# flyakon/DeepPhysiNet

Hardware: AMD Instinct MI355X
Metric: collocation-points/sec (fwd+PDE-Jacobian+bwd) (higher is better)
Workload: dtype bf16x2 (hi+lo split bf16 MFMA operands), fp32 accumulate

## Files before the change

### deepphysinet_amd/csrc/dpn_layout.h

```cpp
#pragma once

#if defined(__HIPCC__)
#define DPN_HD __host__ __device__ constexpr
#else
#define DPN_HD constexpr
#endif

namespace dpn {

constexpr int kNets = 6;
constexpr int kHidden = 256;
constexpr int kPe = 192;
constexpr int kW1Stride = 193;
constexpr int kW2Stride = 257;

DPN_HD int drow32(int r, int h) { return (r & 3) + 8 * (r >> 2) + 4 * h; }
DPN_HD int chain_ch(int ks, int h, int e) { return 16 * ks + 8 * (e >> 2) + 4 * h + (e & 3); }

DPN_HD int pe3_angle(int ks, int h, int e) { return 8 * ks + 4 * h + (e >> 1); }
DPN_HD int pe3_ch(int ks, int h, int e) { return (pe3_angle(ks, h, e) & 31) * 6 + (e & 1) * 3 + (pe3_angle(ks, h, e) >> 5); }
DPN_HD int pe6_ch(int ks, int h, int e) { return (pe3_angle(ks, h, e) & 15) * 12 + (e & 1) * 6 + (pe3_angle(ks, h, e) >> 4); }

DPN_HD int gpe_row_to_pe3_ch(int rho) {
    const int T = rho >> 5, i = rho & 31;
    const int r = (i & 3) + 4 * (i >> 3), h = (i >> 2) & 1;
    return pe3_ch(2 * T + (r >> 3), h, r & 7);
}

constexpr int kS0 = 0;
constexpr int kS1 = kS0 + 8 * 12;
constexpr int kS2 = kS1 + 8 * 28;
constexpr int kS3 = kS2 + 8 * 16;
constexpr int kS4 = kS3 + 8 * 16;
constexpr int kS5 = kS4 + 8 * 16;
constexpr int kPackKB = kS5 + 6 * 16;
enum { kVecB1 = 0, kVecCvec, kVecBf1, kVecU, kVecWo, kVecB2BdE_unused, kNumVecs = 6 };
DPN_HD long pack_bytes_per_net(int ns) { return (long)kPackKB * 1024 * ns + kNumVecs * 1024 + 16; }

constexpr int kF0 = kS0, kFA = kS1, kFB = kS1 + 8 * 16, kFAT = kS2, kF5 = kS5;
static_assert(kFB + 8 * 12 == kS2 && kFAT + 8 * 16 == kS3, "fused form fits the block");
enum { kVecC2 = kVecCvec, kVecA2 = kVecBf1, kVecBv = kVecB2BdE_unused };

}
```

### deepphysinet_amd/csrc/dpn_wgrad.hip

```cpp
#include "dpn_point_common.h"

DEV u16 f2bf(float x) {
    unsigned u = __float_as_uint(x);
    u += 0x7FFFu + ((u >> 16) & 1u);
    return (u16)(u >> 16);
}
DEV float bf2f(u16 b) { return __uint_as_float(((unsigned)b) << 16); }

struct PackArgs {
    DpnNetPtrs net[kNets];
    char* packed;
    int ns;
    int form;
    int n_fields;
    long heads_stride, evec_stride, packed_stride;
};
DEV DpnNetPtrs pack_net(const PackArgs& a, const int net, const int field) {
    DpnNetPtrs P = a.net[net];
    P.w1b1 += field * a.heads_stride;
    P.w2b2 += field * a.heads_stride;
    P.evec += field * a.evec_stride;
    return P;
}

DEV float pack_src(const DpnNetPtrs& P, int kb, int lane, int e) {
    const int i = lane & 31, h = lane >> 5;
    if (kb < kS1) {
        const int T = kb / 12, ks = kb % 12;
        return P.w1b1[(32 * T + i) * P.ld_w1b1 + pe3_ch(ks, h, e)];
    } else if (kb >= kS5) {
        const int rel = kb - kS5, T = rel / 16, ks = rel % 16;
        return P.w1b1[chain_ch(ks, h, e) * P.ld_w1b1 + gpe_row_to_pe3_ch(32 * T + i)];
    }
    if (kb < kS2) {
        const int rel = kb - kS1;
        if (rel < 128) return P.w2b2[(32 * (rel / 16) + i) * P.ld_w2b2 + chain_ch(rel % 16, h, e)];
        const int r2 = rel - 128;
        return P.Wd[(32 * (r2 / 12) + i) * kPe + pe6_ch(r2 % 12, h, e)];
    } else if (kb < kS3) {
        const int rel = kb - kS2, T = rel / 16, ks = rel % 16;
        return P.W1[(32 * T + i) * kHidden + chain_ch(ks, h, e)];
    } else if (kb < kS4) {
        const int rel = kb - kS3, T = rel / 16, ks = rel % 16;
        return P.W1[chain_ch(ks, h, e) * kHidden + (32 * T + i)];
    } else {
        const int rel = kb - kS4, T = rel / 16, ks = rel % 16;
        return P.w2b2[chain_ch(ks, h, e) * P.ld_w2b2 + (32 * T + i)];
    }
}

constexpr int kVecParts = 8;
DEV void pack_vectors(const PackArgs& a, const DpnNetPtrs& P, char* packed_net, const int part) {
    float* vec = reinterpret_cast<float*>(packed_net + (long)kPackKB * 1024 * a.ns);
    const int tid = threadIdx.x, og = tid >> 5;
    const int idx = 32 * part + (tid & 31);
    const int h = idx >> 7, T = (idx >> 4) & 7, r = idx & 15;
    const int ch = 32 * T + drow32(r, h);
    const int c6 = idx < kPe ? pe6_ch(idx >> 4, (idx >> 3) & 1, idx & 7) : 0;
    __shared__ float red[3][8][32];
    float up = 0.f, a2 = 0.f, bv = 0.f;
    if (a.form == 1) {
#pragma unroll 8
        for (int o = 32 * og; o < 32 * og + 32; ++o) {
            const float w = P.wo[o];
            up = fmaf(w, P.W2[o * kHidden + ch], up);
            a2 = fmaf(w, P.w2b2[o * P.ld_w2b2 + ch], a2);
            bv = fmaf(w, P.Wd[o * kPe + c6], bv);
        }
    } else {
#pragma unroll 8
        for (int o = 32 * og; o < 32 * og + 32; ++o) up = fmaf(P.wo[o], P.W2[o * kHidden + ch], up);
    }
    red[0][og][tid & 31] = up; red[1][og][tid & 31] = a2; red[2][og][tid & 31] = bv;
    __syncthreads();
    if (og == 0) {
        const int c = tid;
        auto sum8 = [&](const int q) { return ((red[q][0][c] + red[q][1][c]) + (red[q][2][c] + red[q][3][c])) + ((red[q][4][c] + red[q][5][c]) + (red[q][6][c] + red[q][7][c])); };
        vec[kVecB1 * 256 + idx] = P.w1b1[ch * P.ld_w1b1 + kPe];
        vec[kVecU * 256 + idx] = sum8(0);
        vec[kVecWo * 256 + idx] = P.wo[ch];
        if (a.form == 1) {
            vec[kVecA2 * 256 + idx] = sum8(1);
            vec[kVecBv * 256 + idx] = idx < kPe ? sum8(2) : 0.f;
        } else {
            vec[kVecCvec * 256 + idx] = P.w2b2[ch * P.ld_w2b2 + kHidden] + P.bd[ch] + P.evec[ch];
            vec[kVecBf1 * 256 + idx] = P.bf1[ch];
            vec[kVecB2BdE_unused * 256 + idx] = 0.f;
        }
    }
    if (part != 0) return;
    __shared__ float red1[256];
    const float cv_nat = P.w2b2[tid * P.ld_w2b2 + kHidden] + P.bd[tid] + P.evec[tid];
    red1[tid] = P.wo[tid] * (P.bf2[tid] + (a.form == 1 ? 2.0f * cv_nat : 0.f));
    __syncthreads();
    for (int s = 128; s > 0; s >>= 1) {
        if (tid < s) red1[tid] += red1[tid + s];
        __syncthreads();
    }
    if (tid == 0) {
        vec[kNumVecs * 256 + 0] = red1[0] + P.bo[0];
        vec[kNumVecs * 256 + 1] = (float)a.form; vec[kNumVecs * 256 + 2] = 0.f; vec[kNumVecs * 256 + 3] = 0.f;
    }
}

__global__ __launch_bounds__(256) void dpn_pack_matrices_kernel(PackArgs a) {
    const int mcols = gridDim.x - kVecParts;
    const int field = blockIdx.y / kNets, net = blockIdx.y - field * kNets;
    const int ns = a.ns;
    const DpnNetPtrs P = pack_net(a, net, field);
    char* packed_net = a.packed + field * a.packed_stride + (long)net * pack_bytes_per_net(ns);
    if ((int)blockIdx.x >= mcols) { pack_vectors(a, P, packed_net, blockIdx.x - mcols); return; }
    uint4* dst = reinterpret_cast<uint4*>(packed_net);
    const int total = kPackKB * 64;
    for (int u = blockIdx.x * 256 + threadIdx.x; u < total; u += mcols * 256) {
        const int kb = u >> 6;
        const int lane = u & 63;
        u16 hi[8], lo[8];
#pragma unroll
        for (int e = 0; e < 8; ++e) {
            const float x = pack_src(P, kb, lane, e);
            hi[e] = f2bf(x);
            lo[e] = f2bf(x - bf2f(hi[e]));
        }
        uint4 w;
        w.x = hi[0] | (hi[1] << 16); w.y = hi[2] | (hi[3] << 16); w.z = hi[4] | (hi[5] << 16); w.w = hi[6] | (hi[7] << 16);
        dst[(kb * ns) * 64 + lane] = w;
        if (ns == 2) {
            w.x = lo[0] | (lo[1] << 16); w.y = lo[2] | (lo[3] << 16); w.z = lo[4] | (lo[5] << 16); w.w = lo[6] | (lo[7] << 16);
            dst[(kb * ns + 1) * 64 + lane] = w;
        }
    }
}

constexpr int kFusedBlocks = 64 + 48 + 8 + 12 + kVecParts;
DEV f32x16 pk_mfma_f32(float a, float b, f32x16 c) { return __builtin_amdgcn_mfma_f32_32x32x2f32(a, b, c, 0, 0, 0); }
__global__ __launch_bounds__(256) void dpn_pack_fused_kernel(PackArgs a) {
#ifdef PACK_NO_XCD_REMAP
    const int field = blockIdx.y / kNets, net = blockIdx.y - field * kNets, bx = blockIdx.x, ns = a.ns;
#else
    const int lin = blockIdx.x + kFusedBlocks * blockIdx.y, virt = (lin & 7) * (kFusedBlocks * kNets / 8 * a.n_fields) + (lin >> 3);
    static_assert(kFusedBlocks * kNets % 8 == 0, "remap");
    const int fnet = virt / kFusedBlocks, bx = virt - fnet * kFusedBlocks, ns = a.ns, field = fnet / kNets, net = fnet - field * kNets;
#endif
#ifdef PACK_ABL_MASK
    if (!((PACK_ABL_MASK >> (bx < 64 ? 0 : bx < 112 ? 1 : bx < 120 ? 2 : bx < 132 ? 3 : 4)) & 1)) return;
#endif
    const DpnNetPtrs P = pack_net(a, net, field);
    char* packed_net = a.packed + field * a.packed_stride + (long)net * pack_bytes_per_net(ns);
    if (bx >= 132) { pack_vectors(a, P, packed_net, bx - 132); return; }
    uint4* dst = reinterpret_cast<uint4*>(packed_net);
    auto put = [&](const int kb, const int lane, const float (&x)[8]) __attribute__((always_inline)) {
        u16 hi[8], lo[8];
#pragma unroll
        for (int e = 0; e < 8; ++e) { hi[e] = f2bf(x[e]); lo[e] = f2bf(x[e] - bf2f(hi[e])); }
        uint4 w;
        w.x = hi[0] | (hi[1] << 16); w.y = hi[2] | (hi[3] << 16); w.z = hi[4] | (hi[5] << 16); w.w = hi[6] | (hi[7] << 16);
        dst[(kb * ns) * 64 + lane] = w;
        if (ns == 2) {
            w.x = lo[0] | (lo[1] << 16); w.y = lo[2] | (lo[3] << 16); w.z = lo[4] | (lo[5] << 16); w.w = lo[6] | (lo[7] << 16);
            dst[(kb * ns + 1) * 64 + lane] = w;
        }
    };
    if (bx >= 120) {
        for (int u = (bx - 120) * 256 + threadIdx.x; u < 192 * 64; u += 12 * 256) {
            int kb = u >> 6;
            const int lane = u & 63;
            if (kb >= kS1) kb += kS5 - kS1;
            float x[8];
#pragma unroll
            for (int e = 0; e < 8; ++e) x[e] = pack_src(P, kb, lane, e);
            put(kb, lane, x);
        }
        return;
    }
    const int role = bx < 64 ? 0 : bx < 112 ? 1 : 2;
    const int rb = role == 0 ? bx : role == 1 ? bx - 64 : bx - 112;
    const int To = rb & 7, Tc = role == 2 ? 0 : rb >> 3;
    const int lane = threadIdx.x & 63, wv = threadIdx.x >> 6, col = lane & 31, kh = lane >> 5;
    __shared__ float red[4][16][64];
    __shared__ float tile[32][33];
    const float* W1r = P.W1 + (32 * To + col) * kHidden;
    int ccol = 0;
    if (role == 0) ccol = 32 * Tc + col;
    else if (role == 1) { const int sl = 32 * Tc + col; ccol = pe6_ch(sl >> 4, (sl >> 3) & 1, sl & 7); }
    f32x16 acc = (f32x16)0.f;
    float av[32], bv[32];
#pragma unroll
    for (int m = 0; m < 8; ++m) {
        const int k0 = 64 * wv + 8 * m + 4 * kh;
        const f32x4 q = *reinterpret_cast<const f32x4*>(W1r + k0);
#pragma unroll
        for (int e = 0; e < 4; ++e) {
            const int k = k0 + e;
            av[4 * m + e] = q[e];
            if (role == 0) bv[4 * m + e] = P.w2b2[(long)k * P.ld_w2b2 + ccol];
            else if (role == 1) bv[4 * m + e] = P.Wd[k * kPe + ccol];
            else bv[4 * m + e] = col == 0 ? (P.w2b2[(long)k * P.ld_w2b2 + kHidden] + P.bd[k] + P.evec[k]) : 0.f;
        }
    }
#pragma unroll
    for (int kk = 0; kk < 32; ++kk) acc = pk_mfma_f32(av[kk], bv[kk], acc);
#pragma unroll
    for (int r = 0; r < 16; ++r) red[wv][r][lane] = acc[r];
    __syncthreads();
#pragma unroll
    for (int q = 0; q < 4; ++q) {
        const int r = wv + 4 * q;
        tile[drow32(r, kh)][col] = (red[0][r][lane] + red[1][r][lane]) + (red[2][r][lane] + red[3][r][lane]);
    }
    __syncthreads();
    if (role == 2) {
        if (threadIdx.x < 32) {
            const int o = 32 * To + threadIdx.x, w_ = o & 31;
            float* vec = reinterpret_cast<float*>(packed_net + (long)kPackKB * 1024 * ns);
            vec[kVecC2 * 256 + ((w_ >> 2) & 1) * 128 + (o >> 5) * 16 + (w_ & 3) + 4 * (w_ >> 3)] = tile[threadIdx.x][0] + P.bf1[o];
        }
        return;
    }
    const int form = threadIdx.x >> 7, ksl = (threadIdx.x >> 6) & 1, i = lane & 31, h = lane >> 5;
    float x[8];
    if (role == 1) {
        if (form == 1) return;
#pragma unroll
        for (int e = 0; e < 8; ++e) x[e] = tile[i][16 * ksl + 8 * h + e];
        put(kFB + To * 12 + 2 * Tc + ksl, lane, x);
    } else if (form == 0) {
#pragma unroll
        for (int e = 0; e < 8; ++e) x[e] = tile[i][16 * ksl + 8 * (e >> 2) + 4 * h + (e & 3)];
        put(kFA + To * 16 + 2 * Tc + ksl, lane, x);
    } else {
#pragma unroll
        for (int e = 0; e < 8; ++e) x[e] = tile[16 * ksl + 8 * (e >> 2) + 4 * h + (e & 3)][i];
        put(kFAT + Tc * 16 + 2 * To + ksl, lane, x);
    }
}

constexpr int kPartFloats = 65536 + 49152 * 2 + 7 * 256;
DPN_HD int part_off(int prod) { return prod == 1 ? 0 : prod == 2 ? 65536 : 114688; }
constexpr int kPartVec = 163840;

struct WgradArgs {
    int64_t n, n_pad;
    int splits[4];
    void* saved;
    void* operands;
    float* partials;
#ifdef DPN_WGRAD_PHASES
    unsigned* phases;
#endif
};
#ifdef DPN_WGRAD_PHASES
#define DPN_WG_CLOCK(V) do { unsigned long long t_; asm volatile("s_memtime %0\n\ts_waitcnt lgkmcnt(0)" : "=s"(t_)::"memory"); V = (u32)t_; } while (0)
#else
#define DPN_WG_CLOCK(V) do { } while (0)
#endif

template <int NS, int PROD>
struct WgradShape {
    static constexpr int nct = PROD < 2 ? 8 : 6;
    static constexpr int nsx = PROD == 3 ? NS : 1;
    static constexpr int kX = nsx * 16384, kYPlane = nct * 2048, kY = NS * kYPlane;
    static constexpr int kPieces = (kX + kY) / 1024;
    static constexpr int kIssue = (kPieces + 7) / 8;
    static constexpr int kPad = kIssue * 8 - kPieces;
    static constexpr int kGOff = kX + kY;
    static constexpr int kPadOff = kGOff + 8 * 256;
    static constexpr int kSlot = kPadOff + (kPad ? 1024 : 0);
    static constexpr int PER_TILE = kIssue + 1;
    static constexpr int RING = (160 * 1024) / kSlot < 5 ? (160 * 1024) / kSlot : 5;
};
template <int NS>
constexpr int wgrad_lds_bytes() {
    int m = 0;
    const int v[3] = {WgradShape<NS, 1>::RING * WgradShape<NS, 1>::kSlot, WgradShape<NS, 2>::RING * WgradShape<NS, 2>::kSlot,
                      WgradShape<NS, 3>::RING * WgradShape<NS, 3>::kSlot};
    for (int k = 0; k < 3; ++k) m = v[k] > m ? v[k] : m;
    return m;
}

template <int NS, int PROD>
DEV void wgrad_body(const WgradArgs& a, char* lds, const int split, const int net) {
    using S = WgradShape<NS, PROD>;
    constexpr int nct = S::nct, nsx = S::nsx, kSlot = S::kSlot, RING = S::RING, PER_TILE = S::PER_TILE, ncol = nct * 32;
    const int64_t tiles = a.n_pad / 32;
    const int64_t per = (tiles + a.splits[PROD] - 1) / a.splits[PROD];
    const int64_t t0 = (int64_t)split * per;
    int64_t t1 = t0 + per < tiles ? t0 + per : tiles;
    if (t1 < t0) t1 = t0;

    const int lane = threadIdx.x & 63, wave = __builtin_amdgcn_readfirstlane(threadIdx.x >> 6);
#ifdef DPN_WGRAD_2X4_ONLY
    constexpr bool kWide = true;
#else
    constexpr bool kWide = nct == 8;
#endif
    constexpr int MT = kWide ? 4 : 2, NT = kWide ? 2 : 3;
    const int wm = kWide ? wave >> 2 : wave >> 1, wn = kWide ? wave & 3 : wave & 1;
    const int i = lane & 31, h = lane >> 5;
    const bool active = wn * NT < nct;
    SavedView sv = saved_view(a.saved, a.n_pad, NS);
    OperandView ov = operand_view(a.operands, a.n_pad, NS);
    const char* xb = (PROD == 3) ? sv.T1.base : sv.M2.base;
    static_assert(PROD >= 1 && PROD <= 3, "products: 1 = M2^T Z1, 2 = M2^T G6, 3 = T1^T Z0");
    const char* yb = (PROD == 1) ? ov.Z1.base : (PROD == 2) ? ov.PE6.base : ov.Z0.base;
    const int64_t ynet = (PROD == 2) ? 0 : net;
    const float* gnet = ov.gnet + (int64_t)net * a.n_pad;

    const char* pbase[S::kIssue];
    int pstride[S::kIssue], pdst[S::kIssue];
#pragma unroll
    for (int j = 0; j < S::kIssue; ++j) {
        const int q = wave + 8 * j;
        if (S::kPad && q >= S::kPieces) {
            pbase[j] = xb + ((int64_t)net * nsx * tiles + (t0 < tiles ? t0 : 0)) * 16384; pstride[j] = 0; pdst[j] = S::kPadOff;
        } else if (q < nsx * 16) {
            pbase[j] = xb + ((int64_t)net * nsx + q / 16) * tiles * 16384 + (q % 16) * 1024; pstride[j] = 16384; pdst[j] = q * 1024;
        } else {
            const int qy = q - nsx * 16;
            pbase[j] = yb + (ynet * NS + qy / (2 * nct)) * tiles * S::kYPlane + (qy % (2 * nct)) * 1024; pstride[j] = S::kYPlane; pdst[j] = q * 1024;
        }
    }
    auto issue = [&](int64_t tile, int slot) __attribute__((always_inline)) {
        char* sl = lds + slot * kSlot;
#pragma unroll
        for (int j = 0; j < S::kIssue; ++j) {
            if (PROD == 2 && wave + 8 * j >= nsx * 16) dma16(pbase[j] + tile * pstride[j] + lane * 16, sl + pdst[j]);
            else dma16_nt(pbase[j] + tile * pstride[j] + lane * 16, sl + pdst[j]);
        }
        dma4(reinterpret_cast<const char*>(gnet + tile * 32) + lane * 4, sl + S::kGOff + wave * 256);
    };

    f32x16 acc[MT][NT];
#pragma unroll
    for (int m = 0; m < MT; ++m)
#pragma unroll
        for (int n2 = 0; n2 < NT; ++n2) acc[m][n2] = (f32x16)0.f;
    float vecA[MT], vecB[NT], gsum = 0.f;
#pragma unroll
    for (int m = 0; m < MT; ++m) vecA[m] = 0.f;
#pragma unroll
    for (int n2 = 0; n2 < NT; ++n2) vecB[n2] = 0.f;
    auto owns_row = [&](const int m) __attribute__((always_inline)) { return (kWide && nct == 6) ? wn == m % 3 : wn == m; };
    auto owns_col = [&](const int n2) __attribute__((always_inline)) { return wm == n2; };

    const unsigned lds_base = (unsigned)(uintptr_t)(__attribute__((address_space(3))) char*)lds;
    auto rd128 = [&](u32x4& v, const unsigned addr) __attribute__((always_inline)) {
        asm volatile("ds_read_b128 %0, %1" : "=v"(v) : "v"(addr) : "memory");
    };
    auto compute = [&](const int slot_) __attribute__((always_inline)) {
        const unsigned buf = lds_base + slot_ * kSlot;
        const unsigned gl = buf + S::kGOff + wave * 256;
        constexpr int KB = (NS == 1) ? 2 : 1;
        u32x4 gqa[KB][2], faa[KB][nsx][MT], fba[KB][NS][NT];
        const unsigned baseG = gl + h * 16;
        const unsigned baseA = buf + wm * (MT * 1024) + lane * 16, baseB = buf + S::kX + wn * (NT * 1024) + lane * 16;
        auto rd128o = [&](u32x4& v, const unsigned base, const int off) __attribute__((always_inline)) {
            asm volatile("ds_read_b128 %0, %1 offset:%2" : "=v"(v) : "v"(base), "i"(off) : "memory");
        };
        auto issue_reads = [&](const int kk, const int b) __attribute__((always_inline)) {
            rd128o(gqa[b][0], baseG, 64 * kk);
            rd128o(gqa[b][1], baseG, 64 * kk + 32);
#pragma unroll
            for (int s2 = 0; s2 < nsx; ++s2)
#pragma unroll
                for (int m = 0; m < MT; ++m) rd128o(faa[b][s2][m], baseA, s2 * 16384 + (kk * 8 + m) * 1024);
#pragma unroll
            for (int s2 = 0; s2 < NS; ++s2)
#pragma unroll
                for (int n2 = 0; n2 < NT; ++n2) rd128o(fba[b][s2][n2], baseB, s2 * S::kYPlane + (kk * nct + n2) * 1024);
        };
        constexpr int kReads = 2 + MT * nsx + NT * NS;
        if constexpr (NS == 1) { issue_reads(0, 0); issue_reads(1, 1); }
#pragma unroll
        for (int kk = 0; kk < 2; ++kk) {
            const int b = (NS == 1) ? kk : 0;
            if constexpr (NS == 2) issue_reads(kk, 0);
            u32x4 (&fa)[nsx][MT] = faa[b];
            u32x4 (&fb)[NS][NT] = fba[b];
            u32x4& gq0 = gqa[b][0];
            u32x4& gq1 = gqa[b][1];
            if (NS == 1 && kk == 0) asm volatile("s_waitcnt lgkmcnt(%0)" :: "n"(kReads) : "memory");
            else asm volatile("s_waitcnt lgkmcnt(0)" ::: "memory");
            asm volatile("" : "+v"(gq0), "+v"(gq1), "+v"(fa[0][0]), "+v"(fa[0][1]), "+v"(fb[0][0]), "+v"(fb[0][1]));
            if constexpr (MT == 4) asm volatile("" : "+v"(fa[0][2]), "+v"(fa[0][3]));
            if constexpr (NT == 3) asm volatile("" : "+v"(fb[0][2]));
            if constexpr (NS == 2) asm volatile("" : "+v"(fb[1][0]), "+v"(fb[1][1]));
            if constexpr (NS == 2 && NT == 3) asm volatile("" : "+v"(fb[1][2]));
            if constexpr (nsx == 2) asm volatile("" : "+v"(fa[1][0]), "+v"(fa[1][1]));
            if constexpr (nsx == 2 && MT == 4) asm volatile("" : "+v"(fa[1][2]), "+v"(fa[1][3]));
            const float gp[8] = {__uint_as_float(gq0[0]), __uint_as_float(gq0[1]), __uint_as_float(gq0[2]), __uint_as_float(gq0[3]),
                                 __uint_as_float(gq1[0]), __uint_as_float(gq1[1]), __uint_as_float(gq1[2]), __uint_as_float(gq1[3])};
            if constexpr (PROD == 2) {
#pragma unroll
                for (int n2 = 0; n2 < NT; ++n2)
#pragma unroll
                    for (int p = 0; p < 4; ++p) {
                        float v0 = bf_lo(fb[0][n2][p]), v1 = bf_hi(fb[0][n2][p]);
                        if constexpr (NS == 2) { v0 += bf_lo(fb[1][n2][p]); v1 += bf_hi(fb[1][n2][p]); }
                        const float z0 = gp[2 * p] * v0, z1 = gp[2 * p + 1] * v1;
                        const u32 hi = pack2(z0, z1);
                        fb[0][n2][p] = hi;
                        if constexpr (NS == 2) fb[1][n2][p] = pack2(z0 - bf_lo(hi), z1 - bf_hi(hi));
                    }
            }
            if (PROD == 1 && wave == 0 && i == 0) {
#pragma unroll
                for (int e = 0; e < 8; ++e) gsum += gp[e];
            }
#pragma unroll
            for (int m = 0; m < MT; ++m) {
                if (owns_row(m) && PROD != 2) {
                    float d = 0.f;
#pragma unroll
                    for (int s2 = 0; s2 < nsx; ++s2) {
#pragma unroll
                        for (int p = 0; p < 4; ++p) { d = fmaf(bf_lo(fa[s2][m][p]), gp[2 * p], d); d = fmaf(bf_hi(fa[s2][m][p]), gp[2 * p + 1], d); }
                    }
                    vecA[m] += d;
                }
#pragma unroll
                for (int n2 = 0; n2 < NT; ++n2) {
                    if constexpr (NS == 2) {
                        acc[m][n2] = mfma(as_bf(fa[0][m]), as_bf(fb[1][n2]), acc[m][n2]);
                        if constexpr (nsx == 2) acc[m][n2] = mfma(as_bf(fa[1][m]), as_bf(fb[0][n2]), acc[m][n2]);
                    }
                    acc[m][n2] = mfma(as_bf(fa[0][m]), as_bf(fb[0][n2]), acc[m][n2]);
                }
            }
            if (PROD != 3) {
#pragma unroll
                for (int n2 = 0; n2 < NT; ++n2) {
                    if (!owns_col(n2)) continue;
                    float d = 0.f;
#pragma unroll
                    for (int s2 = 0; s2 < NS; ++s2)
#pragma unroll
                        for (int p = 0; p < 4; ++p) d += bf_lo(fb[s2][n2][p]) + bf_hi(fb[s2][n2][p]);
                    vecB[n2] += d;
                }
            }
        }
    };

    const int64_t tl = t1 > t0 ? t1 - 1 : t0;
#pragma unroll
    for (int r = 0; r < RING - 1; ++r) issue(t0 + r < t1 ? t0 + r : tl, r);
    int slot = 0;
#ifdef DPN_WGRAD_PHASES
    u32 c0 = 0, c1 = 0, c2 = 0, c3 = 0, c4 = 0, ph_wait = 0, ph_bar = 0, ph_issue = 0, ph_comp = 0;
#endif
    for (int64_t tile = t0; tile < t1; ++tile) {
        DPN_WG_CLOCK(c0);
        wait_vmcnt<(RING - 2) * PER_TILE>();
        DPN_WG_CLOCK(c1);
        __builtin_amdgcn_s_barrier();
        DPN_WG_CLOCK(c2);
        {
            const int64_t nt = tile + RING - 1;
            issue(nt < t1 ? nt : tl, (slot + RING - 1) % RING);
        }
        DPN_WG_CLOCK(c3);
        if (active) compute(slot);
        DPN_WG_CLOCK(c4);
#ifdef DPN_WGRAD_PHASES
        ph_wait += c1 - c0; ph_bar += c2 - c1; ph_issue += c3 - c2; ph_comp += c4 - c3;
#endif
        slot = (slot + 1) % RING;
    }
#ifdef DPN_WGRAD_PHASES
    if (a.phases && lane == 0) {
        unsigned* o = a.phases + (((int64_t)blockIdx.y * gridDim.x + blockIdx.x) * 8 + wave) * 8;
        o[0] = ph_wait; o[1] = ph_bar; o[2] = ph_issue; o[3] = ph_comp; o[4] = (unsigned)(t1 - t0); o[5] = PROD;
    }
#endif
    wait_vmcnt<0>();
    __builtin_amdgcn_s_barrier();
    float* part = a.partials + ((int64_t)split * kNets + net) * kPartFloats;
    float* out = part + part_off(PROD);
    if (active) {
#pragma unroll
        for (int m = 0; m < MT; ++m)
#pragma unroll
            for (int n2 = 0; n2 < NT; ++n2)
#pragma unroll
                for (int r = 0; r < 16; ++r) {
                    const int rr = wm * (MT * 32) + 32 * m + drow32(r, h);
                    const int cc = wn * (NT * 32) + 32 * n2 + i;
                    out[rr * ncol + cc] = acc[m][n2][r];
                }
    }
#pragma unroll
    for (int m = 0; m < MT; ++m) {
        const float v = vecA[m] + __shfl_xor(vecA[m], 32);
        if (owns_row(m) && h == 0) {
            const int rr = wm * (MT * 32) + 32 * m + i;
            if (PROD == 1) part[kPartVec + 2 * 256 + rr] = v;
            if (PROD == 3) part[kPartVec + 3 * 256 + rr] = v;
        }
    }
    if (PROD == 1 && wave == 0) {
        const float gs = gsum + __shfl_xor(gsum, 32);
        if (lane == 0) part[kPartVec + 4 * 256] = gs;
    }
    if (PROD != 3 && active) {
        const int qo = kPartVec + (PROD == 1 ? 5 : 6) * 256;
#pragma unroll
        for (int n2 = 0; n2 < NT; ++n2) {
            const float v = vecB[n2] + __shfl_xor(vecB[n2], 32);
            if (owns_col(n2) && h == 0) part[qo + wn * (NT * 32) + 32 * n2 + i] = v;
        }
    }
}

template <int NS>
__global__ __launch_bounds__(512, 2) void dpn_wgrad_kernel(WgradArgs a) {
    __shared__ __attribute__((aligned(16))) char lds[wgrad_lds_bytes<NS>()];
    int prod = 1, split = blockIdx.x;
    const int net = blockIdx.y;
    while (prod < 3 && split >= a.splits[prod]) { split -= a.splits[prod]; ++prod; }
    if (prod == 1) wgrad_body<NS, 1>(a, lds, split, net);
    else if (prod == 2) wgrad_body<NS, 2>(a, lds, split, net);
    else wgrad_body<NS, 3>(a, lds, split, net);
}

struct FinishArgs {
    DpnNetPtrs net[kNets];
    DpnNetGradPtrs grad[kNets];
    const char* packed;
    const float* partials;
    float* scratch_s1;
    float* scratch_s2;
    float* scratch_mv;
    float* scratch_u;
    float* scratch_q1;
    float* scratch_q6;
    float* scratch_sg;
    float* scratch_rp;
    int splits[4], ns;
    int64_t n;
};

DEV int slot_of_ch(int ch) { return (ch & ~15) + 8 * ((ch >> 2) & 1) + 4 * ((ch >> 3) & 1) + (ch & 3); }
DEV int slot_of_pe3(int orig) {
    const int f = orig / 6, fn = (orig % 6) / 3, c = orig % 3;
    const int a = 32 * c + f;
    const int ks = a >> 3, h = (a >> 2) & 1, p = a & 3;
    return 16 * ks + 8 * h + 2 * p + fn;
}
DEV int slot_of_pe6(int orig) {
    const int f = orig / 12, fn = (orig % 12) / 6, c6 = orig % 6;
    const int a = 16 * c6 + f;
    const int ks = a >> 3, h = (a >> 2) & 1, p = a & 3;
    return 16 * ks + 8 * h + 2 * p + fn;
}

constexpr int kMaxSplits = 20;
template <int NQ, int MAXS>
DEV void part_sums_n(const float* partials, const int (&ks)[NQ], int net, const int (&off)[NQ], float (&out)[NQ]) {
    float v[MAXS][NQ];
#pragma unroll
    for (int k = 0; k < MAXS; ++k) {
#pragma unroll
        for (int q = 0; q < NQ; ++q)
            v[k][q] = partials[((int64_t)min(k, ks[q] - 1) * kNets + net) * kPartFloats + off[q]];
    }
#pragma unroll
    for (int q = 0; q < NQ; ++q) {
        float t = 0.f;
#pragma unroll
        for (int k = 0; k < MAXS; ++k) t += (k < ks[q]) ? v[k][q] : 0.f;
        out[q] = t;
    }
}
template <int NQ>
DEV void part_sums(const float* partials, const int (&ks)[NQ], int net, const int (&off)[NQ], float (&out)[NQ]) {
    int most = 0;
#pragma unroll
    for (int q = 0; q < NQ; ++q) most = ks[q] > most ? ks[q] : most;
    if (most <= 12) part_sums_n<NQ, 12>(partials, ks, net, off, out);
    else if (most <= 16) part_sums_n<NQ, 16>(partials, ks, net, off, out);
    else part_sums_n<NQ, kMaxSplits>(partials, ks, net, off, out);
}

__global__ __launch_bounds__(256) void dpn_finish_rows_kernel(FinishArgs a) {
    const int o = blockIdx.x, net = blockIdx.y, i = threadIdx.x;
    const DpnNetGradPtrs& Gd = a.grad[net];
    const int so = slot_of_ch(o), si = slot_of_ch(i);
    float rowv[1] = {0.f};
    const bool has_vec = i < 4 || (i == 4 && o == 0);
    if (has_vec) {
        const int offv[1] = {i == 0 ? kPartVec + 2 * 256 + so : i == 1 ? kPartVec + 3 * 256 + so : i == 2 ? kPartVec + 5 * 256 + so
                             : i == 3 ? kPartVec + 6 * 256 + slot_of_pe6(o < kPe ? o : 0) : kPartVec + 4 * 256};
        const int ksv[1] = {i == 1 ? a.splits[3] : i == 3 ? a.splits[2] : a.splits[1]};
        part_sums<1>(a.partials, ksv, net, offv, rowv);
    }
    if (i < kPe) {
        const int off3[3] = {part_off(1) + so * 256 + si, part_off(2) + so * 192 + slot_of_pe6(i), part_off(3) + so * 192 + slot_of_pe3(i)};
        const int ks3[3] = {a.splits[1], a.splits[2], a.splits[3]};
        float g3[3];
        part_sums<3>(a.partials, ks3, net, off3, g3);
        a.scratch_s1[((int64_t)net * 256 + o) * 256 + i] = g3[0];
        a.scratch_s2[((int64_t)net * 256 + o) * kPe + i] = g3[1];
        Gd.w1b1[o * Gd.ld_w1b1 + i] = g3[2];
    } else {
        const int off1[1] = {part_off(1) + so * 256 + si};
        const int ks1[1] = {a.splits[1]};
        float g1[1];
        part_sums<1>(a.partials, ks1, net, off1, g1);
        a.scratch_s1[((int64_t)net * 256 + o) * 256 + i] = g1[0];
    }
    if (i == 0) {
        const float* vec = reinterpret_cast<const float*>(a.packed + (long)net * pack_bytes_per_net(a.ns) + (long)kPackKB * 1024 * a.ns);
        const int T = o >> 5, w = o & 31, hh = (w >> 2) & 1, r = (w & 3) + 4 * (w >> 3);
        a.scratch_u[net * 256 + o] = vec[kVecU * 256 + hh * 128 + T * 16 + r];
        a.scratch_mv[net * 256 + o] = rowv[0];
    }
    if (i == 1) Gd.w1b1[o * Gd.ld_w1b1 + 192] = rowv[0];
    if (i == 2) a.scratch_q1[net * 256 + o] = rowv[0];
    if (i == 3 && o < kPe) a.scratch_q6[net * 256 + o] = rowv[0];
    if (i == 4 && o == 0) a.scratch_sg[net] = rowv[0];
}

DEV f32x16 mfma_f32_32x32x2(float a, float b, f32x16 c) { return __builtin_amdgcn_mfma_f32_32x32x2f32(a, b, c, 0, 0, 0); }
constexpr int kVsideBlocks = 8 * 15;
DEV void finish_vside_body(const FinishArgs& a, const int bx, const int net, float (&red)[4][16][64], float (&qs)[32]) {
    const int rt = bx & 7, ctile = bx >> 3;
    const int kind = ctile < 8 ? 0 : ctile == 8 ? 1 : 2;
    const DpnNetPtrs& P = a.net[net];
    const DpnNetGradPtrs& Gd = a.grad[net];
    const int lane = threadIdx.x & 63, wv = threadIdx.x >> 6, col = lane & 31, kh = lane >> 5;
    const int o0 = 32 * rt, n0 = kind == 0 ? 32 * ctile : kind == 2 ? 32 * (ctile - 9) : 0, ncol = kind == 0 ? 256 : kind == 2 ? kPe : 1;
    const float* B = kind == 0 ? a.scratch_s1 + (int64_t)net * 65536 : kind == 2 ? a.scratch_s2 + (int64_t)net * 256 * kPe : a.scratch_mv + net * 256;
    const float* U = a.scratch_u + net * 256;
    const int ldb = ncol;
    const bool colok = n0 + col < ncol;
    float qv = 0.f;
    if (wv == 0 && colok) qv = kind == 0 ? a.scratch_q1[net * 256 + n0 + col] : kind == 2 ? a.scratch_q6[net * 256 + n0 + col] : a.scratch_sg[net];
    f32x16 acc = (f32x16)0.f;
    float av[32], bv[32];
#pragma unroll
    for (int kk = 0; kk < 32; ++kk) {
        const int j = 64 * wv + 2 * kk + kh;
        av[kk] = P.W1[j * 256 + o0 + col] * U[j];
        bv[kk] = colok ? B[(int64_t)j * ldb + n0 + col] : 0.f;
    }
#pragma unroll
    for (int kk = 0; kk < 32; ++kk) acc = mfma_f32_32x32x2(av[kk], bv[kk], acc);
#pragma unroll
    for (int r = 0; r < 16; ++r) red[wv][r][lane] = acc[r];
    if (wv == 0 && kh == 0) qs[col] = qv;
    __syncthreads();
#pragma unroll
    for (int q = 0; q < 4; ++q) {
        const int r = wv + 4 * q;
        const float sum = (red[0][r][lane] + red[1][r][lane]) + (red[2][r][lane] + red[3][r][lane]);
        const int o = o0 + drow32(r, kh), i = n0 + col;
        if (!colok) continue;
        const float v = sum + 2.0f * P.wo[o] * qs[col];
        if (kind == 0) Gd.w2b2[o * Gd.ld_w2b2 + i] = v;
        else if (kind == 2) Gd.Wd[o * kPe + i] = v;
        else { Gd.w2b2[o * Gd.ld_w2b2 + 256] = v; Gd.evec[o] = v; Gd.bd[o] = v; }
    }
}

typedef float f32x4u __attribute__((ext_vector_type(4), aligned(4)));
DEV void finish_gside_body(const FinishArgs& a, const int bx, const int net, float (&red)[4][16][64]) {
    const int rt = bx & 7, ct = bx >> 3;
    const DpnNetPtrs& P = a.net[net];
    const DpnNetGradPtrs& Gd = a.grad[net];
    const int lane = threadIdx.x & 63, wv = threadIdx.x >> 6, col = lane & 31, kh = lane >> 5;
    const int o0 = 32 * rt, i0 = 32 * ct;
    const float* S1 = a.scratch_s1 + ((int64_t)net * 256 + o0 + col) * 256;
    const float* S2 = a.scratch_s2 + ((int64_t)net * 256 + o0 + col) * kPe;
    const float* w2 = P.w2b2 + (int64_t)(i0 + col) * P.ld_w2b2;
    const float* Wd = P.Wd + (i0 + col) * kPe;
    f32x4u a1[8], b1[8], a2[6], b2[6];
#pragma unroll
    for (int m = 0; m < 8; ++m) {
        const int k = 64 * wv + 8 * m + 4 * kh;
        a1[m] = *reinterpret_cast<const f32x4u*>(S1 + k);
        b1[m] = *reinterpret_cast<const f32x4u*>(w2 + k);
    }
#pragma unroll
    for (int m = 0; m < 6; ++m) {
        const int k = 48 * wv + 8 * m + 4 * kh;
        a2[m] = *reinterpret_cast<const f32x4u*>(S2 + k);
        b2[m] = *reinterpret_cast<const f32x4u*>(Wd + k);
    }
    f32x16 acc = (f32x16)0.f;
#pragma unroll
    for (int m = 0; m < 8; ++m)
#pragma unroll
        for (int e = 0; e < 4; ++e) acc = mfma_f32_32x32x2(a1[m][e], b1[m][e], acc);
#pragma unroll
    for (int m = 0; m < 6; ++m)
#pragma unroll
        for (int e = 0; e < 4; ++e) acc = mfma_f32_32x32x2(a2[m][e], b2[m][e], acc);
#pragma unroll
    for (int r = 0; r < 16; ++r) red[wv][r][lane] = acc[r];
    __syncthreads();
    const int i = i0 + col;
    const float cv = P.w2b2[(int64_t)i * P.ld_w2b2 + 256] + P.bd[i] + P.evec[i];
#pragma unroll
    for (int q = 0; q < 4; ++q) {
        const int r = wv + 4 * q;
        const int o = o0 + drow32(r, kh);
        const float G = ((red[0][r][lane] + red[1][r][lane]) + (red[2][r][lane] + red[3][r][lane])) + a.scratch_mv[net * 256 + o] * cv;
        Gd.W1[o * 256 + i] = a.scratch_u[net * 256 + o] * G;
        float rp = P.W1[o * 256 + i] * G;
#pragma unroll
        for (int sft = 16; sft > 0; sft >>= 1) rp += __shfl_xor(rp, sft);
        if (col == 0) a.scratch_rp[((int64_t)net * 8 + ct) * 256 + o] = rp;
    }
}

constexpr int kGsideBlocks = 64;
__global__ __launch_bounds__(256) void dpn_finish_sides_kernel(FinishArgs a, int n_v) {
    __shared__ float red[4][16][64];
    __shared__ float qs[32];
#ifdef FINISH_NO_XCD_REMAP
    const int net = blockIdx.y, bx = blockIdx.x;
#else
    const int gx = gridDim.x, total = gx * kNets, lin = blockIdx.x + gx * blockIdx.y, xcd = lin & 7;
    const int virt = xcd * (total >> 3) + min(xcd, total & 7) + (lin >> 3), net = virt / gx, bx = virt - net * gx;
#endif
    if (bx < n_v) finish_vside_body(a, bx, net, red, qs);
    else finish_gside_body(a, bx - n_v, net, red);
}

__global__ __launch_bounds__(256) void dpn_finish_fc2_kernel(FinishArgs a) {
    __shared__ float red[2][256];
    const int net = blockIdx.y, op = blockIdx.x, o = threadIdx.x;
    const DpnNetPtrs& P = a.net[net];
    const DpnNetGradPtrs& Gd = a.grad[net];
    const float* rp = a.scratch_rp + (int64_t)net * 8 * 256 + o;
    const float mv = a.scratch_mv[net * 256 + o];
    const float r = (((rp[0] + rp[256]) + (rp[512] + rp[768])) + ((rp[1024] + rp[1280]) + (rp[1536] + rp[1792]))) + P.bf1[o] * mv;
    const float wop = P.wo[op];
    Gd.W2[op * 256 + o] = wop * r;
    red[0][o] = P.W2[op * 256 + o] * r;
    red[1][o] = a.scratch_q1[net * 256 + o] * P.w2b2[(int64_t)op * P.ld_w2b2 + o] + (o < kPe ? a.scratch_q6[net * 256 + o] * P.Wd[op * kPe + o] : 0.f);
    if (op == 0) Gd.bf1[o] = a.scratch_u[net * 256 + o] * mv;
    __syncthreads();
    for (int s = 128; s > 0; s >>= 1) {
        if (o < s) { red[0][o] += red[0][o + s]; red[1][o] += red[1][o + s]; }
        __syncthreads();
    }
    if (o == 0) {
        const float sg = a.scratch_sg[net];
        const float cv = P.w2b2[(int64_t)op * P.ld_w2b2 + 256] + P.bd[op] + P.evec[op];
        const float zsum = red[1][0] + sg * cv;
        Gd.bf2[op] = wop * sg;
        Gd.wo[op] = red[0][0] + P.bf2[op] * sg + 2.f * zsum;
        if (op == 0) Gd.bo[0] = sg;
    }
}

__global__ void dpn_selftest_kernel(float* out) {
    const int lane = threadIdx.x & 63, i = lane & 31, h = lane >> 5;
    f32x16 acc1 = (f32x16)0.f, acc2 = (f32x16)0.f;
    for (int ks = 0; ks < 2; ++ks) {
        bf16x8 A, B1, B2;
#pragma unroll
        for (int e = 0; e < 8; ++e) {
            const int k = 16 * ks + 8 * h + e;
            A[e] = (__bf16)((k == i) ? 1.f : 0.f);
            B1[e] = (__bf16)(float)k;
            B2[e] = (__bf16)(float)i;
        }
        acc1 = mfma(A, B1, acc1);
        acc2 = mfma(A, B2, acc2);
    }
#pragma unroll
    for (int r = 0; r < 16; ++r) { out[lane * 16 + r] = acc1[r]; out[1024 + lane * 16 + r] = acc2[r]; }
}

struct SplitPlan { int s[4]; int most; };
static inline SplitPlan choose_plan(int64_t n_pad, int ns) {
    int64_t c = n_pad / 32 / 16;
    if (c < 1) c = 1;
    SplitPlan p;
    if (c >= 10) p = (ns == 2) ? SplitPlan{{0, 13, 14, 15}, 15} : SplitPlan{{0, 13, 13, 16}, 16};
    else p = SplitPlan{{0, (int)c, (int)c, (int)c}, (int)c};
#ifdef DPN_EXPERIMENT_SPLITS
    if (const char* e = getenv("DPN_WGRAD_PLAN")) {
        if (sscanf(e, "%d,%d,%d,%d", &p.s[0], &p.s[1], &p.s[2], &p.s[3]) == 4) {
            p.most = 1;
            p.s[0] = 0;
            for (int k = 1; k < 4; ++k) { if (p.s[k] < 1) p.s[k] = 1; if (p.s[k] > kMaxSplits) p.s[k] = kMaxSplits; if (p.s[k] > p.most) p.most = p.s[k]; }
        }
    }
#endif
    return p;
}

__global__ void dpn_clock_stamp_kernel(unsigned long long* ring, unsigned int* cursor, unsigned int cap) {
    const unsigned long long t = wall_clock64();
    ring[atomicAdd(cursor, 1u) % cap] = t;
}

constexpr int64_t kFinishScratchFloats = (int64_t)kNets * 65536 + (int64_t)kNets * 256 * 192 + 4 * kNets * 256 + 8 + (int64_t)kNets * 8 * 256;

extern "C" {

int dpn_version(void) { return 2; }

int dpn_clock_stamp(unsigned long long* ring, unsigned int* cursor, unsigned int cap, void* stream) {
    if (!ring || !cursor || cap == 0) return -1;
    hipLaunchKernelGGL(dpn_clock_stamp_kernel, dim3(1), dim3(1), 0, reinterpret_cast<hipStream_t>(stream), ring, cursor, cap);
    return ck(hipGetLastError());
}

int dpn_clock_rate_khz(int* khz) {
    if (!khz) return -1;
    int dev = 0;
    hipError_t e = hipGetDevice(&dev);
    if (e != hipSuccess) return ck(e);
    return ck(hipDeviceGetAttribute(khz, hipDeviceAttributeWallClockRate, dev));
}

int dpn_fwd_form(int prec, int has_pe_in) { return use_tiles("DPN_FWD_KERNEL", prec, has_pe_in != 0) ? 1 : 0; }

int dpn_sizes(int64_t n, int prec, DpnSizes* out) {
    if (!out || n <= 0 || (prec != 1 && prec != 2)) return -1;
    const int64_t n_pad = pad_points(n);
    out->n_pad = n_pad;
    out->packed = (((int64_t)kNets * pack_bytes_per_net(prec) + 255) / 256) * 256;
    out->saved = saved_state_bytes(n_pad, prec);
    out->operands = operand_bytes(n_pad, prec);
    out->k_splits = choose_plan(n_pad, prec).most;
    out->partials = ((int64_t)out->k_splits * kNets * kPartFloats + kFinishScratchFloats) * 4;
    return 0;
}

int dpn_pack_weights_batch(const DpnNetPtrs nets[DPN_NETS], int n_fields, int64_t heads_stride, int64_t evec_stride, int prec, int form, void* packed,
                           int64_t packed_stride, void* stream) {
    if (!nets || !packed || (prec != 1 && prec != 2) || (form != 0 && form != 1) || n_fields < 1 || n_fields > 65535 / kNets) return -1;
    if (n_fields > 1 && (heads_stride <= 0 || evec_stride <= 0 || packed_stride < (int64_t)kNets * pack_bytes_per_net(prec) || (packed_stride & 15))) return -1;
    PackArgs a;
    for (int k = 0; k < kNets; ++k) a.net[k] = nets[k];
    a.packed = reinterpret_cast<char*>(packed);
    a.ns = prec;
    a.form = form;
    a.n_fields = n_fields; a.heads_stride = heads_stride; a.evec_stride = evec_stride; a.packed_stride = packed_stride;
    hipStream_t s = reinterpret_cast<hipStream_t>(stream);
    if (form == 1) {
        hipLaunchKernelGGL(dpn_pack_fused_kernel, dim3(kFusedBlocks, kNets * n_fields), dim3(256), 0, s, a);
        return ck(hipGetLastError());
    }
    hipLaunchKernelGGL(dpn_pack_matrices_kernel, dim3(40 + kVecParts, kNets * n_fields), dim3(256), 0, s, a);
    return ck(hipGetLastError());
}

int dpn_pack_weights_form(const DpnNetPtrs nets[DPN_NETS], int prec, int form, void* packed, void* stream) {
    return dpn_pack_weights_batch(nets, 1, 0, 0, prec, form, packed, 0, stream);
}

int dpn_pack_weights(const DpnNetPtrs nets[DPN_NETS], int prec, void* packed, void* stream) {
    return dpn_pack_weights_form(nets, prec, dpn_fwd_form(prec, 0), packed, stream);
}

#ifdef DPN_WGRAD_PHASES
static unsigned* g_wgrad_phases = nullptr;
int dpn_debug_set_wgrad_phases(void* buf) { g_wgrad_phases = reinterpret_cast<unsigned*>(buf); return 0; }
#endif
int dpn_wgrad(int64_t n, int prec, const float* g_out, const void* saved, const void* operands, void* partials, void* stream) {
    if (!g_out || !saved || !operands || !partials || n <= 0 || (prec != 1 && prec != 2)) return -1;
    const SplitPlan plan = choose_plan(pad_points(n), prec);
    WgradArgs a{n, pad_points(n), {plan.s[0], plan.s[1], plan.s[2], plan.s[3]}, const_cast<void*>(saved), const_cast<void*>(operands),
                reinterpret_cast<float*>(partials)};
#ifdef DPN_WGRAD_PHASES
    a.phases = g_wgrad_phases;
#endif
    (void)g_out;
    hipStream_t s = reinterpret_cast<hipStream_t>(stream);
    const dim3 grid(plan.s[1] + plan.s[2] + plan.s[3], kNets);
    if (prec == 1) hipLaunchKernelGGL(dpn_wgrad_kernel<1>, grid, dim3(512), 0, s, a);
    else hipLaunchKernelGGL(dpn_wgrad_kernel<2>, grid, dim3(512), 0, s, a);
    return ck(hipGetLastError());
}

int dpn_wgrad_finish_parts(const DpnNetPtrs nets[DPN_NETS], const void* packed, int64_t n, int prec, const void* partials,
                           const DpnNetGradPtrs grads[DPN_NETS], int parts, void* stream) {
    if (!nets || !packed || !partials || !grads || n <= 0 || (prec != 1 && prec != 2) || !(parts & 3)) return -1;
    FinishArgs a;
    for (int k = 0; k < kNets; ++k) { a.net[k] = nets[k]; a.grad[k] = grads[k]; }
    a.packed = reinterpret_cast<const char*>(packed);
    a.partials = reinterpret_cast<const float*>(partials);
    const SplitPlan plan = choose_plan(pad_points(n), prec);
    for (int k = 0; k < 4; ++k) a.splits[k] = plan.s[k];
    a.ns = prec;
    a.n = n;
    a.scratch_s1 = const_cast<float*>(a.partials) + (int64_t)plan.most * kNets * kPartFloats;
    a.scratch_s2 = a.scratch_s1 + (int64_t)kNets * 65536;
    a.scratch_mv = a.scratch_s2 + (int64_t)kNets * 256 * 192;
    a.scratch_u = a.scratch_mv + kNets * 256;
    a.scratch_q1 = a.scratch_u + kNets * 256;
    a.scratch_q6 = a.scratch_q1 + kNets * 256;
    a.scratch_sg = a.scratch_q6 + kNets * 256;
    a.scratch_rp = a.scratch_sg + 8;
    hipStream_t s = reinterpret_cast<hipStream_t>(stream);
    if (parts & 1) hipLaunchKernelGGL(dpn_finish_rows_kernel, dim3(256, kNets), dim3(256), 0, s, a);
    const int n_v = (parts & 1) ? kVsideBlocks : 0, n_g = (parts & 2) ? kGsideBlocks : 0;
    hipLaunchKernelGGL(dpn_finish_sides_kernel, dim3(n_v + n_g, kNets), dim3(256), 0, s, a, n_v);
    if (parts & 2) hipLaunchKernelGGL(dpn_finish_fc2_kernel, dim3(256, kNets), dim3(256), 0, s, a);
    return ck(hipGetLastError());
}

int dpn_wgrad_finish(const DpnNetPtrs nets[DPN_NETS], const void* packed, int64_t n, int prec, const void* partials,
                     const DpnNetGradPtrs grads[DPN_NETS], void* stream) {
    return dpn_wgrad_finish_parts(nets, packed, n, prec, partials, grads, 3, stream);
}

int dpn_selftest(void* scratch_dev, void* stream) {
    if (!scratch_dev) return -1;
    hipStream_t s = reinterpret_cast<hipStream_t>(stream);
    float* out = reinterpret_cast<float*>(scratch_dev);
    hipLaunchKernelGGL(dpn_selftest_kernel, dim3(1), dim3(64), 0, s, out);
    float host[2048];
    if (hipMemcpyAsync(host, out, sizeof(host), hipMemcpyDeviceToHost, s) != hipSuccess) return -2;
    if (hipStreamSynchronize(s) != hipSuccess) return -3;
    for (int lane = 0; lane < 64; ++lane)
        for (int r = 0; r < 16; ++r) {
            const int j = lane & 31, h = lane >> 5, i = drow32(r, h);
            if (host[lane * 16 + r] != (float)i) return 100 + r;
            if (host[1024 + lane * 16 + r] != (float)j) return 200 + r;
        }
    return 0;
}

}
```

Measured before the change: 31.85 million.

## Form gated Y operand cooperatively in LDS once per tile for product 2

For the M2^T G6 weight-gradient product, the g-scaled bf16 hi/lo split of the Y operand used to be recomputed in registers by every wave that read a column tile. Now each wave scales the column pairs it loaded itself and writes them back to LDS before the barrier. Compute then reads the operand already formed. The DMA piece assignment is remapped so each wave owns the Y pieces it forms. This removes redundant per-wave VALU conversion work. In exchange it adds LDS writes, an extra wait before the barrier, and a lopsided split of forming work across waves.

```diff
diff --git a/deepphysinet_amd/csrc/dpn_layout.h b/deepphysinet_amd/csrc/dpn_layout.h
--- a/deepphysinet_amd/csrc/dpn_layout.h
+++ b/deepphysinet_amd/csrc/dpn_layout.h
@@ -41,4 +41,12 @@
 static_assert(kFB + 8 * 12 == kS2 && kFAT + 8 * 16 == kS3, "fused form fits the block");
 enum { kVecC2 = kVecCvec, kVecA2 = kVecBf1, kVecBv = kVecB2BdE_unused };
 
+DPN_HD bool wgrad_coop_is_y(int ns, int wave, int j) { return j < ns || (j < 2 * ns && wave < 4); }
+DPN_HD int wgrad_coop_piece(int ns, int issue, int wave, int j) {
+    const int xlo = issue - 2 * ns, xhi = (16 - 4 * xlo) / 4;
+    if (j < ns) return 16 + 12 * j + wave;
+    if (wave < 4) return j < 2 * ns ? 16 + 12 * (j - ns) + 8 + wave : xlo * wave + (j - 2 * ns);
+    return j - ns < xhi ? 4 * xlo + xhi * (wave - 4) + (j - ns) : -1;
 }
+
+}
diff --git a/deepphysinet_amd/csrc/dpn_wgrad.hip b/deepphysinet_amd/csrc/dpn_wgrad.hip
--- a/deepphysinet_amd/csrc/dpn_wgrad.hip
+++ b/deepphysinet_amd/csrc/dpn_wgrad.hip
@@ -1,3 +1,5 @@
+#include <type_traits>
+
 #include "dpn_point_common.h"
 
 DEV u16 f2bf(float x) {
@@ -306,12 +308,16 @@
     const int64_t ynet = (PROD == 2) ? 0 : net;
     const float* gnet = ov.gnet + (int64_t)net * a.n_pad;
 
+    constexpr bool kCoop = PROD == 2;
+    static_assert(!kCoop || (2 * nct == 12 && nsx == 1 && S::kIssue >= 2 * NS), "product 2: 12 column pairs over 8 waves");
+    const bool two_pairs = wave < 4;
     const char* pbase[S::kIssue];
     int pstride[S::kIssue], pdst[S::kIssue];
 #pragma unroll
     for (int j = 0; j < S::kIssue; ++j) {
-        const int q = wave + 8 * j;
-        if (S::kPad && q >= S::kPieces) {
+        int q = wave + 8 * j;
+        if constexpr (kCoop) q = wgrad_coop_piece(NS, S::kIssue, wave, j);
+        if (S::kPad && (kCoop ? q < 0 : q >= S::kPieces)) {
             pbase[j] = xb + ((int64_t)net * nsx * tiles + (t0 < tiles ? t0 : 0)) * 16384; pstride[j] = 0; pdst[j] = S::kPadOff;
         } else if (q < nsx * 16) {
             pbase[j] = xb + ((int64_t)net * nsx + q / 16) * tiles * 16384 + (q % 16) * 1024; pstride[j] = 16384; pdst[j] = q * 1024;
@@ -324,7 +330,7 @@
         char* sl = lds + slot * kSlot;
 #pragma unroll
         for (int j = 0; j < S::kIssue; ++j) {
-            if (PROD == 2 && wave + 8 * j >= nsx * 16) dma16(pbase[j] + tile * pstride[j] + lane * 16, sl + pdst[j]);
+            if (kCoop && wgrad_coop_is_y(NS, wave, j)) dma16(pbase[j] + tile * pstride[j] + lane * 16, sl + pdst[j]);
             else dma16_nt(pbase[j] + tile * pstride[j] + lane * 16, sl + pdst[j]);
         }
         dma4(reinterpret_cast<const char*>(gnet + tile * 32) + lane * 4, sl + S::kGOff + wave * 256);
@@ -358,8 +364,10 @@
             asm volatile("ds_read_b128 %0, %1 offset:%2" : "=v"(v) : "v"(base), "i"(off) : "memory");
         };
         auto issue_reads = [&](const int kk, const int b) __attribute__((always_inline)) {
-            rd128o(gqa[b][0], baseG, 64 * kk);
-            rd128o(gqa[b][1], baseG, 64 * kk + 32);
+            if constexpr (!kCoop) {
+                rd128o(gqa[b][0], baseG, 64 * kk);
+                rd128o(gqa[b][1], baseG, 64 * kk + 32);
+            }
 #pragma unroll
             for (int s2 = 0; s2 < nsx; ++s2)
 #pragma unroll
@@ -369,7 +377,7 @@
 #pragma unroll
                 for (int n2 = 0; n2 < NT; ++n2) rd128o(fba[b][s2][n2], baseB, s2 * S::kYPlane + (kk * nct + n2) * 1024);
         };
-        constexpr int kReads = 2 + MT * nsx + NT * NS;
+        constexpr int kReads = (kCoop ? 0 : 2) + MT * nsx + NT * NS;
         if constexpr (NS == 1) { issue_reads(0, 0); issue_reads(1, 1); }
 #pragma unroll
         for (int kk = 0; kk < 2; ++kk) {
@@ -381,7 +389,9 @@
             u32x4& gq1 = gqa[b][1];
             if (NS == 1 && kk == 0) asm volatile("s_waitcnt lgkmcnt(%0)" :: "n"(kReads) : "memory");
             else asm volatile("s_waitcnt lgkmcnt(0)" ::: "memory");
-            asm volatile("" : "+v"(gq0), "+v"(gq1), "+v"(fa[0][0]), "+v"(fa[0][1]), "+v"(fb[0][0]), "+v"(fb[0][1]));
+            if constexpr (kCoop) gq0 = gq1 = (u32x4)0u;
+            else asm volatile("" : "+v"(gq0), "+v"(gq1));
+            asm volatile("" : "+v"(fa[0][0]), "+v"(fa[0][1]), "+v"(fb[0][0]), "+v"(fb[0][1]));
             if constexpr (MT == 4) asm volatile("" : "+v"(fa[0][2]), "+v"(fa[0][3]));
             if constexpr (NT == 3) asm volatile("" : "+v"(fb[0][2]));
             if constexpr (NS == 2) asm volatile("" : "+v"(fb[1][0]), "+v"(fb[1][1]));
@@ -390,19 +400,6 @@
             if constexpr (nsx == 2 && MT == 4) asm volatile("" : "+v"(fa[1][2]), "+v"(fa[1][3]));
             const float gp[8] = {__uint_as_float(gq0[0]), __uint_as_float(gq0[1]), __uint_as_float(gq0[2]), __uint_as_float(gq0[3]),
                                  __uint_as_float(gq1[0]), __uint_as_float(gq1[1]), __uint_as_float(gq1[2]), __uint_as_float(gq1[3])};
-            if constexpr (PROD == 2) {
-#pragma unroll
-                for (int n2 = 0; n2 < NT; ++n2)
-#pragma unroll
-                    for (int p = 0; p < 4; ++p) {
-                        float v0 = bf_lo(fb[0][n2][p]), v1 = bf_hi(fb[0][n2][p]);
-                        if constexpr (NS == 2) { v0 += bf_lo(fb[1][n2][p]); v1 += bf_hi(fb[1][n2][p]); }
-                        const float z0 = gp[2 * p] * v0, z1 = gp[2 * p + 1] * v1;
-                        const u32 hi = pack2(z0, z1);
-                        fb[0][n2][p] = hi;
-                        if constexpr (NS == 2) fb[1][n2][p] = pack2(z0 - bf_lo(hi), z1 - bf_hi(hi));
-                    }
-            }
             if (PROD == 1 && wave == 0 && i == 0) {
 #pragma unroll
                 for (int e = 0; e < 8; ++e) gsum += gp[e];
@@ -442,6 +439,39 @@
         }
     };
 
+    auto form = [&](const int slot_) __attribute__((always_inline)) {
+        const unsigned buf = lds_base + slot_ * kSlot;
+        const unsigned baseG = buf + S::kGOff + wave * 256 + h * 16, baseY = buf + S::kX + wave * 1024 + lane * 16;
+        auto pair = [&](auto q_) __attribute__((always_inline)) {
+            constexpr int q = decltype(q_)::value;
+            const unsigned ay = baseY + q * 8192, ag = baseG + ((wave + 8 * q) >= nct ? 64 : 0);
+            u32x4 t[2], gq0, gq1;
+            rd128(gq0, ag);
+            asm volatile("ds_read_b128 %0, %1 offset:32" : "=v"(gq1) : "v"(ag) : "memory");
+            rd128(t[0], ay);
+            if constexpr (NS == 2) asm volatile("ds_read_b128 %0, %1 offset:%2" : "=v"(t[1]) : "v"(ay), "i"(S::kYPlane) : "memory");
+            asm volatile("s_waitcnt lgkmcnt(0)" ::: "memory");
+            asm volatile("" : "+v"(gq0), "+v"(gq1), "+v"(t[0]));
+            if constexpr (NS == 2) asm volatile("" : "+v"(t[1]));
+            const float gp[8] = {__uint_as_float(gq0[0]), __uint_as_float(gq0[1]), __uint_as_float(gq0[2]), __uint_as_float(gq0[3]),
+                                 __uint_as_float(gq1[0]), __uint_as_float(gq1[1]), __uint_as_float(gq1[2]), __uint_as_float(gq1[3])};
+#pragma unroll
+            for (int p = 0; p < 4; ++p) {
+                float v0 = bf_lo(t[0][p]), v1 = bf_hi(t[0][p]);
+                if constexpr (NS == 2) { v0 += bf_lo(t[1][p]); v1 += bf_hi(t[1][p]); }
+                const float z0 = gp[2 * p] * v0, z1 = gp[2 * p + 1] * v1;
+                const u32 hi = pack2(z0, z1);
+                t[0][p] = hi;
+                if constexpr (NS == 2) t[1][p] = pack2(z0 - bf_lo(hi), z1 - bf_hi(hi));
+            }
+            asm volatile("ds_write_b128 %0, %1" :: "v"(ay), "v"(t[0]) : "memory");
+            if constexpr (NS == 2) asm volatile("ds_write_b128 %0, %1 offset:%2" :: "v"(ay), "v"(t[1]), "i"(S::kYPlane) : "memory");
+        };
+        pair(std::integral_constant<int, 0>{});
+        if (two_pairs) pair(std::integral_constant<int, 1>{});
+        asm volatile("s_waitcnt lgkmcnt(0)" ::: "memory");
+    };
+
     const int64_t tl = t1 > t0 ? t1 - 1 : t0;
 #pragma unroll
     for (int r = 0; r < RING - 1; ++r) issue(t0 + r < t1 ? t0 + r : tl, r);
@@ -452,6 +482,7 @@
     for (int64_t tile = t0; tile < t1; ++tile) {
         DPN_WG_CLOCK(c0);
         wait_vmcnt<(RING - 2) * PER_TILE>();
+        if constexpr (kCoop) form(slot);
         DPN_WG_CLOCK(c1);
         __builtin_amdgcn_s_barrier();
         DPN_WG_CLOCK(c2);
```

Result: faster. 32.33 million, median of 6 (+1.5%).
